# merbanan/rtl_433

Measured on NVIDIA H100. Metric: IQ MS/s end-to-end demod+slice, higher is better.
Workload: dtype u8/int16/int32 fixed point

## Files before the change

rtl_433_b200/csrc/r433b_api.cu:

```cuda
#include <algorithm>
#include <cmath>
#include <cstdio>
#include <cstdlib>
#include <chrono>
#include <cstring>
#include <exception>
#include <atomic>
#include <mutex>
#include <string>
#include <thread>
#include <vector>

#include "../../include/r433b.h"
#include "../../include/r433b_abi.h"
#include "r433b_kernels.cuh"
#include "r433b_host.hpp"
#include "r433b_pulses.hpp"
#include "r433b_analyze.cuh"
#include "r433b_analyze_host.hpp"
#include "r433b_grab.cuh"

using namespace r433b;

#ifdef R433B_SIMT_EMU
// ... 859 lines not shown
    ctx->timing.front_redone = counters[4];
    ctx->timing.front_repairs = counters[5];
    ctx->timing.idle_skipped = counters[6];
    ctx->timing.idle_rewalks = counters[7];
    ctx->timing.chain_folds = counters[8];
    ctx->timing.chain_fm_rebuilds = counters[9];
    cudaEventElapsedTime(&ctx->timing.total_ms, ctx->ev[0], ctx->ev[3]);
    ctx->timing.d2h_ms = 0;
    ctx->timing.detect_launches = detect_launches;
    ctx->processed = true;
    finish_chain();
    return R433B_OK;
}

}

int r433b_process(r433b_ctx *ctx, r433b_batch const *b) { return process_iq(ctx, b, nullptr, nullptr); }

int r433b_chain_create(r433b_ctx *ctx, uint32_t n_streams, r433b_chain **out)
{
    if (!ctx || !out || !n_streams) return fail(ctx, R433B_EINVAL, "r433b_chain_create: null argument or no streams");
    *out = nullptr;
    CU(cudaSetDevice(ctx->device));
    r433b_chain *ch = new (std::nothrow) r433b_chain();
    if (!ch) return R433B_ENOMEM;
    ch->ctx = ctx;
    ctx->chains.push_back(ch);
    ch->n = n_streams;
    ch->open.assign(n_streams, 0);
    ch->next.assign(n_streams, 0);
    size_t const n = n_streams;
    for (auto [buf, bytes] : {std::pair<DevBuf *, size_t>{&ch->d_state, n * sizeof(StreamState)}, {&ch->d_state_copy, n * sizeof(StreamState)},
                              {&ch->d_train, n * kTrainInts * sizeof(int)}, {&ch->d_train_copy, n * kTrainInts * sizeof(int)},
                              {&ch->d_flags, 2 * n}, {&ch->d_base, n * sizeof(uint64_t)}})
        if (int r = dev_reserve(ctx, *buf, bytes)) {
            r433b_chain_destroy(ch);
            return r;
        }
    *out = ch;
    return R433B_OK;
}

void r433b_chain_destroy(r433b_chain *ch)
{
    if (!ch) return;
    if (r433b_ctx *ctx = ch->ctx) {
        ctx->chains.erase(std::remove(ctx->chains.begin(), ctx->chains.end(), ch), ctx->chains.end());
        cudaSetDevice(ctx->device);
        chain_free_device(ch);
    }
    delete ch;
}

int r433b_process_chained(r433b_ctx *ctx, r433b_batch const *b, r433b_chain *chain, uint8_t const *last)
{
    if (!chain || !chain->ctx) return fail(ctx, R433B_EINVAL, "r433b_process_chained: no chain, or its context is gone");
    return process_iq(ctx, b, chain, last);
}

int r433b_chain_base(r433b_chain const *chain, uint32_t stream, uint64_t *first_sample)
{
    if (!chain || !first_sample || stream >= chain->n) return R433B_EINVAL;
    *first_sample = stream < chain->base.size() ? chain->base[stream] : 0;
    return R433B_OK;
}

int r433b_get_counts(r433b_ctx const *ctx, uint64_t out[4])
{
    if (!ctx || !out) return R433B_EINVAL;
    if (!ctx->processed) return R433B_ESTATE;
    out[0] = ctx->n_pkgs;
    out[1] = ctx->n_events;
    out[2] = ctx->event_bytes;
    out[3] = ctx->n_samples;
    return R433B_OK;
}

int r433b_get_timing(r433b_ctx const *ctx, r433b_timing *out)
{
    if (!ctx || !out) return R433B_EINVAL;
    *out = ctx->timing;
    return R433B_OK;
}

int r433b_fetch(r433b_ctx *ctx, r433b_results *out)
{
    if (!ctx || !out) return R433B_EINVAL;
    if (!ctx->processed) return fail(ctx, R433B_ESTATE, "r433b_fetch before r433b_process");
    CU(cudaSetDevice(ctx->device));
    cudaStream_t const st = 0;
    uint32_t const n_devs = (uint32_t)ctx->devs.size();
    size_t pk_bytes = (size_t)ctx->n_pkgs * sizeof(r433b_package);
    size_t pool_bytes = (size_t)ctx->pool_used * sizeof(int);
    size_t pair_bytes = (size_t)ctx->n_pkgs * n_devs * sizeof(r433b_pair);
    CU(cudaEventRecord(ctx->ev[4], st));
    if (int r = host_reserve(ctx, ctx->h_pkgs, pk_bytes + 16)) return r;
    if (int r = host_reserve(ctx, ctx->h_ppool, pool_bytes + 16)) return r;
    if (int r = host_reserve(ctx, ctx->h_gpool, pool_bytes + 16)) return r;
    if (int r = host_reserve(ctx, ctx->h_pairs, pair_bytes + 16)) return r;
    if (int r = host_reserve(ctx, ctx->h_events, ctx->event_bytes + 16)) return r;
    if (!ctx->d2h_done) {
        if (pk_bytes) CU(cudaMemcpyAsync(ctx->h_pkgs.p, ctx->d_pkgs.p, pk_bytes, cudaMemcpyDeviceToHost, st));
        if (pool_bytes) {
            CU(cudaMemcpyAsync(ctx->h_ppool.p, ctx->d_ppool.p, pool_bytes, cudaMemcpyDeviceToHost, st));
            CU(cudaMemcpyAsync(ctx->h_gpool.p, ctx->d_gpool.p, pool_bytes, cudaMemcpyDeviceToHost, st));
        }
        if (pair_bytes && ctx->d_pairs.p) CU(cudaMemcpyAsync(ctx->h_pairs.p, ctx->d_pairs.p, pair_bytes, cudaMemcpyDeviceToHost, st));
        if (ctx->event_bytes) CU(cudaMemcpyAsync(ctx->h_events.p, ctx->d_arena.p, ctx->event_bytes, cudaMemcpyDeviceToHost, st));
        ctx->d2h_done = true;
    }
    CU(cudaEventRecord(ctx->ev[5], st));
    CU(cudaEventSynchronize(ctx->ev[5]));
    cudaEventElapsedTime(&ctx->timing.d2h_ms, ctx->ev[4], ctx->ev[5]);
    r433b_package *pk = (r433b_package *)ctx->h_pkgs.p;
    if (!ctx->fetched) {
        std::vector<uint32_t> &ix = ctx->dev_index;
        ix.resize(ctx->n_pkgs);
        for (uint32_t i = 0; i < ctx->n_pkgs; ++i) ix[i] = i;
        std::sort(ix.begin(), ix.end(), [pk](uint32_t a, uint32_t b) {
            return pk[a].stream != pk[b].stream ? pk[a].stream < pk[b].stream : pk[a].seq < pk[b].seq;
        });
        std::vector<r433b_package> sorted(ctx->n_pkgs);
        for (uint32_t i = 0; i < ctx->n_pkgs; ++i) sorted[i] = pk[ix[i]];
        if (ctx->n_pkgs) memcpy(pk, sorted.data(), (size_t)ctx->n_pkgs * sizeof(r433b_package));
        ctx->analyzed = false;
        ctx->p_events.assign(ctx->n_pkgs, 0);
        ctx->dispatched.assign(ctx->batch.n_streams, 0);
    }
    ctx->fetched = true;
    out->n_packages = ctx->n_pkgs;
    out->n_devices = n_devs;
    out->packages = pk;
    out->pulse_pool = (int32_t const *)ctx->h_ppool.p;
    out->gap_pool = (int32_t const *)ctx->h_gpool.p;
    out->pairs = (r433b_pair const *)ctx->h_pairs.p;
    out->events = (uint8_t const *)ctx->h_events.p;
    out->event_bytes = ctx->event_bytes;
    out->n_events = ctx->n_events;
    out->n_samples = ctx->n_samples;
    out->n_gated = ctx->n_gated;
    return R433B_OK;
}

int r433b_copy_stage(r433b_ctx *ctx, uint32_t stream, int16_t *am, int16_t *fm, uint64_t max_samples)
{
    if (!ctx || !am || !fm) return R433B_EINVAL;
    if (!ctx->processed || !ctx->batch.want_stages) return fail(ctx, R433B_ESTATE, "no stage arrays kept (batch.want_stages)");
    if (stream >= ctx->batch.n_streams) return fail(ctx, R433B_EINVAL, "stream out of range");
    CU(cudaSetDevice(ctx->device));
    uint64_t SS = ctx->batch.sample_format;
    uint64_t first = ctx->offsets[stream] / SS;
    uint64_t n = ctx->lengths[stream] / SS;
    if (n > max_samples) n = max_samples;
    if (n) {
        CU(cudaMemcpy(am, (int16_t const *)ctx->d_am.p + ctx->am_offsets[stream], n * sizeof(int16_t), cudaMemcpyDeviceToHost));
        CU(cudaMemcpy(fm, (int16_t const *)ctx->d_fm.p + first, n * sizeof(int16_t), cudaMemcpyDeviceToHost));
    }
    return (int)std::min<uint64_t>(n, 0x7fffffff);
}


int r433b_event_to_bitbuffer(uint8_t const *ev, uint32_t pair_bytes, uint32_t index, struct bitbuffer *out,
        uint32_t *consumed)
{
    return event_to_bitbuffer(ev, pair_bytes, index, out, consumed);
}

float r433b_package_file_pos(r433b_ctx const *ctx, r433b_results const *res, uint32_t package)
{
    if (!ctx || !res || package >= res->n_packages) return 0.0f;
    if (ctx->pulse_mode) return 0.0f;
    r433b_package const &k = res->packages[package];
    uint64_t SS = ctx->batch.sample_format;
    uint64_t bytes = ctx->lengths[k.stream] + (ctx->chained ? ctx->chain_base[k.stream] * SS : 0);
    uint32_t bb = ctx->batch.block_bytes;
    uint64_t n_blocks = (bytes + bb - 1) / bb;
    if (n_blocks == 0) return 0.0f;
    uint64_t blk = (uint64_t)k.block < n_blocks ? (uint64_t)k.block : n_blocks - 1;
    unsigned long n_read = (unsigned long)std::min<uint64_t>(bb, bytes - blk * bb);
    float pos = ((float)(int)blk * bb + n_read) / ctx->batch.samp_rate / (int)SS;
    return pos;
}

int r433b_package_to_pulse_data(r433b_ctx const *ctx, r433b_results const *res, uint32_t package, struct pulse_data *pd)
{
    if (!ctx || !res || !pd || package >= res->n_packages) return R433B_EINVAL;
    r433b_package const &k = res->packages[package];
    memset(pd, 0, sizeof(*pd));
    if (ctx->pulse_mode) {
        if (k.end_pos >= ctx->pulse_meta.size()) return R433B_EINVAL;
        PulseSet::Meta const &m = ctx->pulse_meta[k.end_pos];
        pd->sample_rate = m.rate;
        pd->num_pulses = m.num_pulses;
        memcpy(pd->pulse, res->pulse_pool + k.pulse_off, k.pulse_count * sizeof(int));
        memcpy(pd->gap, res->gap_pool + k.pulse_off, k.pulse_count * sizeof(int));
        pd->fsk_f1_est = m.fsk_f1_est;
        pd->fsk_f2_est = m.fsk_f2_est;
        pd->freq1_hz = m.freq1_hz;
        pd->freq2_hz = m.freq2_hz;
        return R433B_OK;
    }
    pd->offset = k.offset;
    pd->sample_rate = ctx->batch.samp_rate;
    pd->start_ago = k.start_ago;
    pd->end_ago = k.end_ago;
    pd->num_pulses = k.num_pulses;
    memcpy(pd->pulse, res->pulse_pool + k.pulse_off, k.pulse_count * sizeof(int));
    memcpy(pd->gap, res->gap_pool + k.pulse_off, k.pulse_count * sizeof(int));
    pd->ook_low_estimate = k.ook_low_estimate;
    pd->ook_high_estimate = k.ook_high_estimate;
    pd->fsk_f1_est = k.fsk_f1_est;
    pd->fsk_f2_est = k.fsk_f2_est;
    float hi = pd->ook_high_estimate > 0 ? pd->ook_high_estimate : 1;
    float lo = pd->ook_low_estimate > 0 ? pd->ook_low_estimate : 1;
    int const max_high = ctx->lv.max_high;
    float top = hi < max_high ? hi : max_high;
    float asnr = top / lo;
    uint32_t rate = ctx->batch.samp_rate, center = ctx->batch.center_frequency;
    float off1 = (float)pd->fsk_f1_est / INT16_MAX * rate / 2.0f;
    float off2 = (float)pd->fsk_f2_est / INT16_MAX * rate / 2.0f;
    pd->freq1_hz = off1 + center;
    pd->freq2_hz = off2 + center;
    pd->centerfreq_hz = center;
    pd->depth_bits = ctx->batch.sample_format * 4;
    if (ctx->batch.sample_format == 2 && !ctx->use_mag) {
        pd->range_db = 42.1442f;
        pd->rssi_db = 10.0f * log10f(hi) - 42.1442f;
        pd->noise_db = 10.0f * log10f(lo) - 42.1442f;
        pd->snr_db = 10.0f * log10f(asnr);
    } else {
        pd->range_db = 84.2884f;
        pd->rssi_db = 20.0f * log10f(hi) - 84.2884f;
        pd->noise_db = 20.0f * log10f(lo) - 84.2884f;
        pd->snr_db = 20.0f * log10f(asnr);
    }
    return R433B_OK;
}

}

namespace {

template <class PerEvent, class PerPair>
int replay_stream(r433b_ctx *ctx, r433b_results const *res, uint32_t stream, PerEvent &&per_event, PerPair &&per_pair)
{
    if (!ctx || !res) return R433B_EINVAL;
    if (!ctx->fetched) return fail(ctx, R433B_ESTATE, "dispatch before fetch");
    uint32_t const n_devs = res->n_devices;
    r433b_package const *begin = std::lower_bound(res->packages, res->packages + res->n_packages, stream,
            [](r433b_package const &k, uint32_t s) { return k.stream < s; });
    static thread_local struct pulse_data pd;
    static thread_local struct bitbuffer bits;
    for (r433b_package const *k = begin; k != res->packages + res->n_packages && k->stream == stream; ++k) {
        uint32_t pi = (uint32_t)(k - res->packages);
        r433b_package_to_pulse_data(ctx, res, pi, &pd);
        int p_events = 0;
        unsigned next = 0;
        for (unsigned prio = 0; !p_events && prio < 0xffffffffu; prio = next) {
            next = 0xffffffffu;
            for (uint32_t dv = 0; dv < n_devs; ++dv) {
                unsigned dp = ctx->devs[dv].priority;
                if (dp > prio && dp < next) next = dp;
                if (dp != prio) continue;
                if (!device_takes((int)ctx->devs[dv].modulation, k->type)) continue;
                r433b_pair const &pr = res->pairs[(size_t)k->first_pair + dv];
                per_pair(dv, pr);
                uint32_t at = 0;
                for (uint32_t e = 0; e < pr.events; ++e) {
                    uint32_t used = 0;
                    int rc = r433b_event_to_bitbuffer(res->events + pr.offset + at, pr.bytes - at, 0, &bits, &used);
                    if (rc) return fail(ctx, rc, "corrupt event stream");
                    at += used;
                    int ret = per_event(pi, dv, &pd, &bits);
                    if (ret < -4) return fail(ctx, R433B_EINVAL, "decoder returned an invalid code (< -4)");
                    if (ret > 0) p_events += ret;
                }
            }
        }
        if (pi < ctx->p_events.size()) ctx->p_events[pi] = (uint32_t)p_events;
    }
    if (stream < ctx->dispatched.size()) ctx->dispatched[stream] = 1;
    return R433B_OK;
}

}

extern "C" {

int r433b_stream_digest(r433b_ctx *ctx, r433b_results const *res, uint32_t stream, uint64_t *digest)
{
    if (!ctx || !res || !digest) return R433B_EINVAL;
    if (!ctx->fetched) return fail(ctx, R433B_ESTATE, "digest before fetch");
    uint64_t h = 1469598103934665603ull;
    auto mix = [&](uint32_t w) {
        h ^= w;
        h *= 1099511628211ull;
    };
    auto mix_words = [&](void const *ptr, size_t n_words) {
        uint32_t const *w = (uint32_t const *)ptr;
        for (size_t i = 0; i < n_words; ++i) mix(w[i]);
    };
    r433b_package const *begin = std::lower_bound(res->packages, res->packages + res->n_packages, stream,
            [](r433b_package const &k, uint32_t s) { return k.stream < s; });
    for (r433b_package const *k = begin; k != res->packages + res->n_packages && k->stream == stream; ++k) {
        uint32_t const hdr[] = {k->seq, (uint32_t)k->type, (uint32_t)k->block, (uint32_t)k->offset, (uint32_t)(k->offset >> 32),
                                ctx->pulse_mode ? 0u : (uint32_t)k->end_pos, ctx->pulse_mode ? 0u : (uint32_t)(k->end_pos >> 32), k->start_ago, k->end_ago, k->num_pulses,
                                k->pulse_count, (uint32_t)k->ook_low_estimate, (uint32_t)k->ook_high_estimate,
                                (uint32_t)k->fsk_f1_est, (uint32_t)k->fsk_f2_est};
        mix_words(hdr, sizeof(hdr) / 4);
        mix_words(res->pulse_pool + k->pulse_off, k->pulse_count);
        mix_words(res->gap_pool + k->pulse_off, k->pulse_count);
        for (uint32_t dv = 0; dv < res->n_devices; ++dv) {
            r433b_pair const &pr = res->pairs[(size_t)k->first_pair + dv];
            mix(pr.bytes);
            mix(pr.events);
            mix(pr.gated_single);
            mix(pr.gated_multi);
            if (pr.bytes) mix_words(res->events + pr.offset, pr.bytes / 4);
        }
    }
    *digest = h;
    return R433B_OK;
}

int r433b_dispatch(r433b_ctx *ctx, r433b_results const *res, uint32_t stream, r433b_event_fn fn, void *user)
{
    if (!fn) return R433B_EINVAL;
    return replay_stream(ctx, res, stream, [&](uint32_t pk, uint32_t dv, struct pulse_data *pd, struct bitbuffer *bits) {
        return fn(user, pk, dv, pd, bits);
    }, [](uint32_t, r433b_pair const &) {});
}

int r433b_dispatch_r_devices(r433b_ctx *ctx, r433b_results const *res, uint32_t stream, struct r_device *const *devs,
        uint32_t n)
{
    if (!devs || !res || n != res->n_devices) return R433B_EINVAL;
    return replay_stream(ctx, res, stream, [&](uint32_t, uint32_t dv, struct pulse_data *, struct bitbuffer *bits) {
        struct r_device *d = devs[dv];
        int ret = 0;
        if (d->decode_fn) ret = d->decode_fn(d, bits);
        d->decode_events += 1;
        if (ret > 0) {
            d->decode_ok += 1;
            d->decode_messages += ret;
        } else if (ret >= -4) {
            d->decode_fails[-ret] += 1;
            ret = 0;
        }
        return ret;
    }, [&](uint32_t dv, r433b_pair const &pr) {
        if (!(pr.gated_single | pr.gated_multi) || ctx->gates.size() != n) return;
        struct r_device *d = devs[dv];
        r433b_gate const &g = ctx->gates[dv];
        d->decode_events += pr.gated_single + pr.gated_multi;
        d->decode_fails[-g.code_single] += pr.gated_single;
        d->decode_fails[-g.code_multi] += pr.gated_multi;
    });
}

}

extern "C" {

int r433b_dispatch_r_devices_parallel(r433b_ctx *ctx, r433b_results const *res, struct r_device *const *const *dev_sets,
        uint32_t n_devs, uint32_t n_sets)
{
    if (!ctx || !res || !dev_sets || !n_sets || n_devs != res->n_devices) return R433B_EINVAL;
    if (!ctx->fetched) return fail(ctx, R433B_ESTATE, "dispatch before fetch");
    uint32_t const n_streams = res->n_packages ? res->packages[res->n_packages - 1].stream + 1 : 0;
    std::atomic<int> first_error{0};
    auto work = [&](uint32_t w) {
        for (uint32_t s = w; s < n_streams && !first_error.load(std::memory_order_relaxed); s += n_sets) {
            int rc = r433b_dispatch_r_devices(ctx, res, s, dev_sets[w], n_devs);
            if (rc) {
                int expected = 0;
                first_error.compare_exchange_strong(expected, rc);
            }
        }
    };
    std::vector<std::thread> pool;
    for (uint32_t w = 1; w < n_sets; ++w) pool.emplace_back(work, w);
    work(0);
    for (auto &t : pool) t.join();
    return first_error.load();
}

}


extern "C" {

r433b_pulses *r433b_pulses_create(void) { return new (std::nothrow) r433b_pulses(); }

void r433b_pulses_destroy(r433b_pulses *ps) { delete ps; }

void r433b_pulses_clear(r433b_pulses *ps)
{
    if (!ps) return;
    ps->set = PulseSet();
}

int r433b_pulses_load_ook(r433b_pulses *ps, uint32_t stream, char const *text, size_t len, uint32_t samp_rate)
{
    if (!ps || (!text && len) || !samp_rate) return R433B_EINVAL;
    return load_ook_text(ps->set, stream, text, len, samp_rate);
}

int r433b_pulses_load_rfraw(r433b_pulses *ps, uint32_t stream, char const *line)
{
    if (!ps || !line) return R433B_EINVAL;
    if (!rfraw_is(line)) return 0;
    static thread_local struct pulse_data d;
    memset(&d, 0, sizeof(d));
    rfraw_append(&d, line);
    ps->set.add(stream, &d);
    return 1;
}

int r433b_pulses_add(r433b_pulses *ps, uint32_t stream, struct pulse_data const *pd)
{
    if (!ps || !pd) return R433B_EINVAL;
    ps->set.add(stream, pd);
    return 1;
}

uint32_t r433b_pulses_count(r433b_pulses const *ps) { return ps ? (uint32_t)ps->set.pk.size() : 0; }

int r433b_pulses_get(r433b_pulses const *ps, uint32_t index, struct pulse_data *out)
{
    if (!ps || !out || index >= ps->set.pk.size()) return R433B_EINVAL;
    ps->set.get(index, out);
    return R433B_OK;
}

size_t r433b_format_ook(struct pulse_data const *pd, char const *received, char *buf, size_t cap)
{
    return pd ? format_ook(pd, received, buf, cap) : 0;
}

size_t r433b_format_ook_header(char const *created, char *buf, size_t cap) { return format_ook_header(created, buf, cap); }

size_t r433b_format_vcd(struct pulse_data const *pd, int ch_id, char *buf, size_t cap)
{
    return pd ? format_vcd(pd, ch_id, buf, cap) : 0;
}

size_t r433b_format_vcd_header(uint32_t sample_rate, char const *date, char *buf, size_t cap)
{
    return format_vcd_header(sample_rate, date, buf, cap);
}

void r433b_dump_logic_u8(uint8_t *buf, uint64_t len, uint64_t buf_offset, struct pulse_data const *pd, uint8_t bits)
{
    if (buf && pd) dump_logic_u8(buf, len, buf_offset, pd, bits);
}

int r433b_process_pulses(r433b_ctx *ctx, r433b_pulses const *ps)
{
    if (!ctx || !ps) return fail(ctx, R433B_EINVAL, "null argument");
    CU(cudaSetDevice(ctx->device));
    PulseSet const &set = ps->set;
    uint32_t const n = (uint32_t)set.pk.size();
    uint32_t const n_devs = (uint32_t)ctx->devs.size();
    if ((uint64_t)n * n_devs > 0xffffffffull)
        return fail(ctx, R433B_EOVERFLOW, "packages x devices exceeds the 32-bit pair index (r433b_package.first_pair)");
    ctx->processed = ctx->fetched = false;
    ctx->d2h_done = false;
    ctx->pulse_mode = true;
    ctx->grab_planned = false;
    ctx->pulse_meta = set.pk;
    ctx->batch = r433b_batch{};
    ctx->batch.sample_format = 2;
    ctx->offsets.clear();
    ctx->lengths.clear();
    cudaStream_t const st = 0;

    std::vector<uint32_t> order(n);
    for (uint32_t i = 0; i < n; ++i) order[i] = i;
    std::stable_sort(order.begin(), order.end(), [&](uint32_t a, uint32_t b) { return set.pk[a].rate < set.pk[b].rate; });
    std::vector<r433b_package> hp(n);
    std::vector<int32_t> pp, gp;
    pp.reserve(set.pulse.size());
    gp.reserve(set.gap.size());
    std::vector<uint32_t> rates;
    std::vector<GroupRange> ranges;
    for (uint32_t j = 0; j < n; ++j) {
        PulseSet::Meta const &m = set.pk[order[j]];
        r433b_package &k = hp[j];
        memset(&k, 0, sizeof(k));
        k.stream = m.stream;
        k.seq = m.seq;
        k.type = m.type;
        k.end_pos = order[j];
        k.num_pulses = m.num_pulses;
        k.pulse_off = (uint32_t)pp.size();
        k.pulse_count = m.count;
        k.fsk_f1_est = m.fsk_f1_est;
        k.fsk_f2_est = m.fsk_f2_est;
        k.first_pair = j * n_devs;
        pp.insert(pp.end(), set.pulse.begin() + m.first, set.pulse.begin() + m.first + m.count);
        gp.insert(gp.end(), set.gap.begin() + m.first, set.gap.begin() + m.first + m.count);
        if (rates.empty() || rates.back() != m.rate) {
            rates.push_back(m.rate);
            ranges.push_back(GroupRange{});
            ranges.back().pkg_begin = j;
        }
        ranges.back().pkg_end = j + 1;
    }
    for (uint32_t rate : rates)
        if (!rate) return fail(ctx, R433B_EINVAL, "a package has sample_rate 0");

    ctx->n_pkgs = n;
    ctx->pool_used = (unsigned)pp.size();
    ctx->n_samples = 0;
    ctx->event_bytes = ctx->n_events = ctx->n_gated = 0;
    ctx->timing = r433b_timing{};
    if (n) {
        if (int r = dev_reserve(ctx, ctx->d_pkgs, (size_t)n * sizeof(r433b_package))) return r;
        if (int r = dev_reserve(ctx, ctx->d_ppool, pp.size() * sizeof(int) + 16)) return r;
        if (int r = dev_reserve(ctx, ctx->d_gpool, gp.size() * sizeof(int) + 16)) return r;
        CU(cudaMemcpyAsync(ctx->d_pkgs.p, hp.data(), (size_t)n * sizeof(r433b_package), cudaMemcpyHostToDevice, st));
        CU(cudaMemcpyAsync(ctx->d_ppool.p, pp.data(), pp.size() * sizeof(int), cudaMemcpyHostToDevice, st));
        CU(cudaMemcpyAsync(ctx->d_gpool.p, gp.data(), gp.size() * sizeof(int), cudaMemcpyHostToDevice, st));
        CU(cudaStreamSynchronize(st));
    }
    if (n && n_devs) {
        size_t const arena_min = ctx->min_caps[2] ? ctx->min_caps[2] : (size_t)(1u << 20);
        if (ctx->arena_cap < arena_min) ctx->arena_cap = arena_min;
        if (int r = upload_slicer_tables(ctx, rates, st)) return r;
        if (int r = slice_ranges(ctx, ranges, n, st)) return r;
        ctx->timing.total_ms = ctx->timing.slice_ms;
    }
    ctx->processed = true;
    return R433B_OK;
}

}



namespace {

uint32_t package_rate(r433b_ctx const *ctx, r433b_package const &k)
{
    if (ctx->pulse_mode && k.end_pos < ctx->pulse_meta.size()) return ctx->pulse_meta[k.end_pos].rate;
    return ctx->batch.samp_rate;
}

}

extern "C" {

int r433b_analyze(r433b_ctx *ctx, r433b_results const *res)
{
    if (!ctx || !res) return R433B_EINVAL;
    if (!ctx->fetched) return fail(ctx, R433B_ESTATE, "r433b_analyze before r433b_fetch");
    CU(cudaSetDevice(ctx->device));
    uint32_t const n = ctx->n_pkgs;
    ctx->an.assign(n, r433b_analysis{});
    ctx->an_guess.assign(n, r433b_guess{});
    ctx->an_text.assign(n, std::string());
    ctx->an_pairs.assign(n, r433b_pair{});
    ctx->an_events.clear();
    ctx->analyzed = true;
    if (!n) return R433B_OK;
    cudaStream_t const st = 0;
    if (int r = dev_reserve(ctx, ctx->d_an, (size_t)n * sizeof(r433b_analysis))) return r;
    AnalyzeParams ap{};
    ap.pkgs = (r433b_package const *)ctx->d_pkgs.p;
    ap.n_pkgs = n;
    ap.pulse_pool = (int const *)ctx->d_ppool.p;
    ap.gap_pool = (int const *)ctx->d_gpool.p;
    ap.out = (r433b_analysis *)ctx->d_an.p;
    unsigned const grid = (unsigned)(((uint64_t)n * 5 + kAnalyzeThreads - 1) / kAnalyzeThreads);
    R4_LAUNCH(k_analyze, grid, kAnalyzeThreads, 0, st, ap);
    CU(cudaGetLastError());
    CU(cudaMemcpyAsync(ctx->an.data(), ctx->d_an.p, (size_t)n * sizeof(r433b_analysis), cudaMemcpyDeviceToHost, st));
    CU(cudaStreamSynchronize(st));
    std::vector<SlicerParams> sp(n);
    std::vector<int> last_gap(n, -1);
    static thread_local struct pulse_data pd;
    std::vector<char> buf(1 << 16);
    bool any = false;
    for (uint32_t i = 0; i < n; ++i) {
        uint32_t const di = ctx->dev_index[i];
        r433b_package_to_pulse_data(ctx, res, i, &pd);
        r433b_guess g{};
        size_t len = analysis_finish(&pd, res->packages[i].type, ctx->an[di], &g, buf.data(), buf.size());
        if (len >= buf.size()) {
            buf.resize(len + 1);
            len = analysis_finish(&pd, res->packages[i].type, ctx->an[di], &g, buf.data(), buf.size());
        }
        ctx->an_text[di].assign(buf.data(), len);
        ctx->an_guess[di] = g;
        sp[di] = SlicerParams{};
        if (g.modulation && g.sliced) {
            r433b_device d{};
            d.modulation = g.modulation;
            d.short_width = g.short_width;
            d.long_width = g.long_width;
            d.reset_limit = g.reset_limit;
            d.gap_limit = g.gap_limit;
            d.sync_width = g.sync_width;
            d.tolerance = g.tolerance;
            sp[di] = scale_device(d, package_rate(ctx, res->packages[i]));
            last_gap[di] = g.last_gap;
            any = true;
        }
    }
    if (!any) return R433B_OK;
    if (int r = dev_reserve(ctx, ctx->d_an_dev, (size_t)n * sizeof(SlicerParams))) return r;
    if (int r = dev_reserve(ctx, ctx->d_an_gap, (size_t)n * sizeof(int))) return r;
    if (int r = dev_reserve(ctx, ctx->d_an_pairs, (size_t)n * sizeof(r433b_pair))) return r;
    CU(cudaMemcpyAsync(ctx->d_an_dev.p, sp.data(), (size_t)n * sizeof(SlicerParams), cudaMemcpyHostToDevice, st));
    CU(cudaMemcpyAsync(ctx->d_an_gap.p, last_gap.data(), (size_t)n * sizeof(int), cudaMemcpyHostToDevice, st));
    CU(cudaMemsetAsync(ctx->d_an_pairs.p, 0, (size_t)n * sizeof(r433b_pair), st));
    OwnSliceParams op{};
    op.pkgs = ap.pkgs;
    op.n_pkgs = n;
    op.pulse_pool = ap.pulse_pool;
    op.gap_pool = (int *)ctx->d_gpool.p;
// ... 321 lines not shown
```

rtl_433_b200/csrc/r433b_host.hpp:

```cpp
#pragma once
#include <algorithm>
#include <cmath>
#include <cstdint>
#include <cstring>
#include <vector>

#include "../../include/r433b.h"
#include "../../include/r433b_abi.h"
#include "r433b_core.cuh"
#include "r433b_slice.cuh"

namespace r433b {

inline Levels compute_levels(int use_mag, float level_limit, float min_level, float min_snr)
{
    Levels lv;
    if (use_mag) {
        lv.fixed_high = level_limit < 0.0 ? (int)(powf(10, (level_limit + 84.2884f) / 20.0f)) : 0;
        lv.min_high = (int)(powf(10, (min_level + 84.2884f) / 20.0f));
        lv.ratio = (int)(0.5 + powf(10, min_snr / 20.0f));
    } else {
        lv.fixed_high = level_limit < 0.0 ? (int)(powf(10, (level_limit + 42.1442f) / 10.0f)) : 0;
        lv.min_high = (int)(powf(10, (min_level + 42.1442f) / 10.0f));
        lv.ratio = (int)(0.5 + powf(10, min_snr / 10.0f));
    }
    lv.max_high = (int)(powf(10, (0 + 42.1442f) / 10.0f));
    return lv;
}

inline void fm_coeffs(int cs16, uint32_t rate, float low_pass, int &a1, int &b0)
{
    if (low_pass > 1e4f)
        low_pass = low_pass / rate;
    else if (low_pass >= 1.0f)
        low_pass = 1e6f / low_pass / rate;
    double ita = 1.0 / tan(M_PI_2 * low_pass);
    if (!cs16) {
        double gain = 1.0 / (1.0 + ita) / 2;
        a1 = (int)((ita - 1.0) * gain * 32768);
        b0 = (int)(gain * 32768);
    } else {
        double gain = 1.0 / (1.0 + ita);
        a1 = (int)((ita - 1.0) * gain * (1 << 30));
        b0 = (int)(gain * (1 << 30));
    }
}

inline SlicerParams scale_device(r433b_device const &d, uint32_t rate)
{
    SlicerParams t{};
    float per_us = rate / 1.0e6f;
    t.modulation = (int)d.modulation;
    t.s_short = d.short_width * per_us;
    t.s_long = d.long_width * per_us;
    t.s_reset = d.reset_limit * per_us;
    t.s_gap = d.gap_limit * per_us;
    t.s_sync = d.sync_width * per_us;
    t.s_tol = d.tolerance * per_us;
    bool bad3 = (d.short_width > 0 && t.s_short <= 0) || (d.long_width > 0 && t.s_long <= 0)
            || (d.reset_limit > 0 && t.s_reset <= 0);
    bool bad6 = bad3 || (d.gap_limit > 0 && t.s_gap <= 0) || (d.sync_width > 0 && t.s_sync <= 0)
            || (d.tolerance > 0 && t.s_tol <= 0);
    t.ok = (bad6 ? 0 : 1) | (bad3 ? 0 : 2);
    if ((int)d.modulation == kModOokRzi) {
        t.s_gap = t.s_sync = t.s_tol = 0;
    }
    t.f_short = d.short_width > 0.0f ? 1.0f / (d.short_width * per_us) : 0;
    t.f_long = d.long_width > 0.0f ? 1.0f / (d.long_width * per_us) : 0;
    t.priority = d.priority;
    return t;
}


inline std::vector<unsigned> slice_list(std::vector<r433b_device> const &devs, int package_type)
{
    std::vector<unsigned> v;
    for (unsigned i = 0; i < (unsigned)devs.size(); ++i)
        if (device_takes((int)devs[i].modulation, package_type)) v.push_back(i);
    std::sort(v.begin(), v.end(), [&](unsigned a, unsigned c) {
        r433b_device const &x = devs[a], &y = devs[c];
        if (x.modulation != y.modulation) return x.modulation < y.modulation;
        if (x.reset_limit != y.reset_limit) return x.reset_limit < y.reset_limit;
        if (x.short_width != y.short_width) return x.short_width < y.short_width;
        return a < c;
    });
    return v;
}


inline int event_to_bitbuffer(uint8_t const *ev8, uint32_t pair_bytes, uint32_t index, struct bitbuffer *out,
        uint32_t *consumed)
{
    if (!ev8 || !out || (pair_bytes & 3)) return -1;
    uint32_t const *ev = reinterpret_cast<uint32_t const *>(ev8);
    uint32_t const total = pair_bytes / 4;
    uint32_t pos = 0;
    for (uint32_t i = 0;; ++i) {
        if (pos + 1 > total) return -1;
        uint32_t h = ev[pos];
        uint32_t num_rows = h & 0x7f, dirty = (h >> 7) & 1, free_row = (h >> 8) & 0xff, len = h >> 16;
        if (len < 1 || pos + len > total) return -1;
        if (i == index) {
            memset(out, 0, sizeof(*out));
            out->num_rows = (uint16_t)num_rows;
            out->free_row = (uint16_t)free_row;
            uint32_t q = pos + 1;
            uint32_t const end = pos + len;
            uint8_t *flat = &out->bb[0][0];
            for (uint32_t r = 0; r < num_rows && r < R433B_BITBUF_ROWS; ++r) {
                if (q + 1 > end) return -1;
                uint32_t bits = ev[q] & 0xffff, syncs = ev[q] >> 16;
                q += 1;
                uint32_t words = (bits + 31) / 32;
                if (dirty && r + 1 == num_rows) words = ev[end - 1];
                if (q + words > end) return -1;
                out->bits_per_row[r] = (uint16_t)bits;
                out->syncs_before_row[r] = (uint16_t)syncs;
                size_t at = (size_t)r * R433B_BITBUF_COLS;
                size_t room = sizeof(out->bb) - at;
                size_t nb = (size_t)words * 4;
                memcpy(flat + at, ev + q, nb < room ? nb : room);
                q += words;
            }
            if (consumed) *consumed = (pos + len) * 4;
            return 0;
        }
        pos += len;
    }
}

}
```

rtl_433_b200/csrc/r433b_slice.cuh:

```cuda
#pragma once
#include <stdint.h>
#include "r433b_core.cuh"

namespace r433b {

constexpr int kBbRows = 50;
constexpr int kBbCols = 128;

#ifdef __CUDA_ARCH__
R4_HD float fmul(float a, float b) { return __fmul_rn(a, b); }
R4_HD float fadd(float a, float b) { return __fadd_rn(a, b); }
R4_HD float fdiv(float a, float b) { return __fdiv_rn(a, b); }
R4_HD double dadd(double a, double b) { return __dadd_rn(a, b); }
R4_HD double dmul(double a, double b) { return __dmul_rn(a, b); }
#else
R4_HD float fmul(float a, float b) { volatile float r = a * b; return r; }
R4_HD float fadd(float a, float b) { volatile float r = a + b; return r; }
R4_HD float fdiv(float a, float b) { volatile float r = a / b; return r; }
R4_HD double dadd(double a, double b) { volatile double r = a + b; return r; }
R4_HD double dmul(double a, double b) { volatile double r = a * b; return r; }
#endif

struct SlicerParams {
    int modulation;
    int ok;
    int s_short, s_long, s_reset, s_gap, s_sync, s_tol;
    float f_short, f_long;
    unsigned priority;
    int gate;
};


R4_HD uint32_t bswap32(uint32_t v)
{
#ifdef __CUDA_ARCH__
    return __byte_perm(v, 0, 0x0123);
#else
    return (v >> 24) | ((v >> 8) & 0xff00u) | ((v << 8) & 0xff0000u) | (v << 24);
#endif
}

#ifndef R4_SLICE_WINDOW
#define R4_SLICE_WINDOW 16
#endif
constexpr unsigned kSliceWindow = R4_SLICE_WINDOW;
static_assert(kSliceWindow >= 8 && (kSliceWindow & (kSliceWindow - 1)) == 0, "the window is a power of two of >= 1 sector");
struct NoWindow { static constexpr bool kOn = false; };

template <class Win>
R4_HD unsigned window_slide(uint32_t *out, unsigned wb, unsigned at)
{
    unsigned const b = (at + 8 - kSliceWindow) & ~7u;
    unsigned const end = b < wb + kSliceWindow ? b : wb + kSliceWindow;
    for (unsigned s = wb; s < end; s += 8) {
        uint32_t v[8];
#pragma unroll
        for (int k = 0; k < 8; ++k) v[k] = Win::slot((s + k) % kSliceWindow);
#ifdef __CUDA_ARCH__
        reinterpret_cast<uint4 *>(out + s)[0] = make_uint4(v[0], v[1], v[2], v[3]);
        reinterpret_cast<uint4 *>(out + s)[1] = make_uint4(v[4], v[5], v[6], v[7]);
#else
        for (int k = 0; k < 8; ++k) out[s + k] = v[k];
#endif
    }
    return b;
}

template <class Win = NoWindow>
struct EventWriterT {
    uint32_t *out;
    unsigned limit;
    unsigned wb;

    unsigned pos;
    unsigned committed;
    unsigned events;
    unsigned ev_start;
    unsigned num_rows, free_row;
    unsigned row0_bits;
    unsigned row_hdr;
    unsigned bits, syncs;
    unsigned row_hw;
    uint32_t acc;
    bool dirty;
    unsigned gate;
    unsigned max_bits;
    unsigned gated1, gatedN;

    R4_HD void init(uint32_t *o, unsigned region_words = 0, unsigned gate_bits = 0)
    {
        out = o;
        limit = region_words;
        wb = 0;
        pos = committed = 0;
        events = 0;
        gate = gate_bits;
        gated1 = gatedN = 0;
        reset_event();
    }

    R4_HD void reset_event()
    {
        pos = committed;
        ev_start = committed;
        num_rows = free_row = 0;
        row0_bits = 0;
        row_hdr = 0;
        bits = syncs = row_hw = 0;
        acc = 0;
        dirty = false;
        max_bits = 0;
        if constexpr (Win::kOn) {
            if (committed < wb) {
                unsigned const b = committed & ~7u;
                for (unsigned q = b; q < committed; ++q) Win::slot(q % kSliceWindow) = out[q];
                wb = b;
            }
        }
    }

    R4_HD void put(unsigned at, uint32_t v)
    {
        if (!out || at >= limit) return;
        if constexpr (Win::kOn) {
            if (at >= wb + kSliceWindow) wb = window_slide<Win>(out, wb, at);
            if (at >= wb) {
                Win::slot(at % kSliceWindow) = v;
                return;
            }
        }
        out[at] = v;
    }

    R4_HD uint32_t get(unsigned at) const
    {
        if constexpr (Win::kOn) {
            if (at >= wb) return Win::slot(at % kSliceWindow);
        }
        return out[at];
    }

    R4_HD unsigned first_row_bits() const { return num_rows <= 1 ? bits : row0_bits; }
    R4_HD unsigned last_row_bits() const { return bits; }

    R4_HD void open_row()
    {
        row_hdr = pos;
        pos += 1;
        bits = syncs = row_hw = 0;
        acc = 0;
    }

    R4_HD void flush_word()
    {
        unsigned w = (bits - 1) >> 5;
        unsigned at = row_hdr + 1 + w;
        if (out && at < limit) {
            uint32_t v = bswap32(acc);
            if (w < row_hw) v |= get(at);
            put(at, v);
        }
        if (w + 1 > row_hw) row_hw = w + 1;
        acc = 0;
    }

    R4_HD void close_row()
    {
        if (bits & 31) flush_word();
        put(row_hdr, bits | (syncs << 16));
        pos = row_hdr + 1 + row_hw;
    }

    R4_HD void first_row()
    {
        if (num_rows == 0) {
            ev_start = pos;
            pos += 1;
            num_rows = free_row = 1;
            open_row();
        }
    }

    R4_HD void add_bits(int value, int count)
    {
        first_row();
        {
            unsigned const p = bits & 31, in_row = bits & (kBbCols * 8 - 1);
            if ((unsigned)count <= 32 - p && (in_row != 0 || bits == 0) && bits < 60000u) {
                if (value) acc |= (0xffffffffu >> (32 - count)) << (32 - p - count);
                bits += (unsigned)count;
                if ((bits & 31) == 0) flush_word();
                return;
            }
        }
        while (count > 0) {
            if (bits == 65535u) return;
            if (bits > 0 && (bits & (kBbCols * 8 - 1)) == 0) {
                if (free_row < (unsigned)kBbRows)
                    free_row++;
                else
                    return;
            }
            unsigned p = bits & 31;
            unsigned room = 32 - p;
            unsigned n = (unsigned)count < room ? (unsigned)count : room;
            if (bits + n > 65535u) n = 65535u - bits;
            if (value) acc |= (n == 32 ? 0xffffffffu : ((1u << n) - 1u)) << (room - n);
            bits += n;
            count -= (int)n;
            if ((bits & 31) == 0) flush_word();
        }
    }

    R4_HD void add_bit(int bit) { add_bits(bit, 1); }

    R4_HD void add_row()
    {
        first_row();
        if (free_row < (unsigned)kBbRows) {
            if (num_rows == 1) row0_bits = bits;
            if (bits > max_bits) max_bits = bits;
            close_row();
            free_row++;
            for (unsigned r = num_rows; r + 1 < free_row; ++r) {
                put(pos, 0);
                pos += 1;
            }
            num_rows = free_row;
            open_row();
        } else {
            if (bits & 31) flush_word();
            bits = 0;
            dirty = true;
            acc = 0;
        }
    }

    R4_HD void add_sync()
    {
        first_row();
        if (bits) add_row();
        syncs++;
    }

    R4_HD void emit()
    {
        if (num_rows == 0) {
            ev_start = pos;
            pos += 1;
        } else if ((bits > max_bits ? bits : max_bits) < gate) {
            if (num_rows == 1) gated1++; else gatedN++;
            reset_event();
            return;
        } else {
            close_row();
            if (dirty) {
                put(pos, row_hw);
                pos += 1;
            }
        }
        put(ev_start, num_rows | (dirty ? 0x80u : 0u) | (free_row << 8) | ((pos - ev_start) << 16));
        committed = pos;
        events++;
        reset_event();
    }
};
using EventWriter = EventWriterT<>;


struct PulseView {
    int const *pulse;
    int const *gap;
    unsigned n;
};

enum {
    kModOokMc = 3, kModOokPcm = 4, kModOokPpm = 5, kModOokPwm = 6, kModOokPiwmRaw = 8, kModOokDmc = 9,
    kModOokOsv1 = 10, kModOokPiwmDc = 11, kModOokNrzs = 12, kModOokRzi = 13,
    kModFskPcm = 16, kModFskPwm = 17, kModFskMc = 18
};

R4_HD bool device_takes(int modulation, int package_type)
{
    if (package_type == 1) return modulation >= 3 && modulation <= 13 && modulation != 7;
    return modulation >= 16 && modulation <= 18;
}

R4_HD int iabs(int v) { return v < 0 ? -v : v; }
R4_HD bool within(int v, int nominal, int tol) { return v >= nominal - tol && v <= nominal + tol; }
R4_HD int symbol_at(PulseView const &p, unsigned k) { return (k & 1) ? p.gap[k >> 1] : p.pulse[k >> 1]; }

enum { kRowNone = 0, kRowAdd, kRowSync, kRowClear, kRowIfOpen };
enum { kEmitNone = 0, kEmitAlways, kEmitIfRows, kEmitIfData, kEmitIfRow0, kEmitElseRowIfOpen };
struct Step {
    int ones;
    int zeros;
    int row;
    int bit;
    int emit;
    bool stop_if_emitted, clear_after;
    int post_zeros;
};

struct SlicerState {
    unsigned k, total;
    int b0, b1, b2, b3, b4, b5;
    float f_short, f_long;
    int i0, i1, i2;
    int since;
    double edge;
    bool pending;
    int cv, cg;
};

R4_HD void slicer_advance(PulseView const &p, SlicerState &st, unsigned k)
{
    st.k = k;
    if (k < st.total) {
        st.cv = p.pulse[k];
        st.cg = p.gap[k];
    }
}

constexpr int kModAny = -1;
template <int MOD>
R4_HD int slicer_family(SlicerParams const &t)
{
    if (MOD != kModAny) return MOD;
    int const m = t.modulation;
    return m == kModFskPwm ? (int)kModOokPwm : m == kModFskPcm ? (int)kModOokPcm : m == kModFskMc ? (int)kModOokMc : m;
}

template <int MOD>
R4_HD bool slicer_begin0(PulseView const &p, SlicerParams const &t, SlicerState &st)
{
    st.k = 0;
    st.cv = st.cg = 0;
    st.total = p.n;
    st.since = 0;
    st.pending = false;
    int const big = 0x7fffffff;
    switch (slicer_family<MOD>(t)) {
    case kModOokPwm: {
        if (!(t.ok & 1)) return false;
        st.b4 = st.b5 = 0;
        if (t.s_tol > 0) {
            st.b0 = t.s_short - t.s_tol; st.b1 = t.s_short + t.s_tol;
            st.b2 = t.s_long - t.s_tol;  st.b3 = t.s_long + t.s_tol;
            if (t.s_sync > 0) { st.b4 = t.s_sync - t.s_tol; st.b5 = t.s_sync + t.s_tol; }
        } else if (t.s_sync <= 0) {
            st.b0 = 0; st.b1 = (t.s_short + t.s_long) / 2 + 1;
            st.b2 = st.b1 - 1; st.b3 = big;
        } else if (t.s_sync < t.s_short) {
            st.b4 = 0; st.b5 = (t.s_sync + t.s_short) / 2 + 1;
            st.b0 = st.b5 - 1; st.b1 = (t.s_short + t.s_long) / 2 + 1;
            st.b2 = st.b1 - 1; st.b3 = big;
        } else if (t.s_sync < t.s_long) {
            st.b0 = 0; st.b1 = (t.s_short + t.s_sync) / 2 + 1;
            st.b4 = st.b1 - 1; st.b5 = (t.s_sync + t.s_long) / 2 + 1;
            st.b2 = st.b5 - 1; st.b3 = big;
        } else {
            st.b0 = 0; st.b1 = (t.s_short + t.s_long) / 2 + 1;
            st.b2 = st.b1 - 1; st.b3 = (t.s_long + t.s_sync) / 2 + 1;
            st.b4 = st.b3 - 1; st.b5 = big;
        }
        return true;
    }
    case kModOokPpm: {
        if (!(t.ok & 1)) return false;
        st.b4 = st.b5 = 0;
        if (t.s_tol > 0) {
            st.b0 = t.s_short - t.s_tol; st.b1 = t.s_short + t.s_tol;
            st.b2 = t.s_long - t.s_tol;  st.b3 = t.s_long + t.s_tol;
            if (t.s_sync > 0) { st.b4 = t.s_sync - t.s_tol; st.b5 = t.s_sync + t.s_tol; }
        } else {
            st.b0 = 0;
            st.b1 = (t.s_short + t.s_long) / 2 + 1;
            st.b2 = st.b1 - 1;
            st.b3 = t.s_gap ? t.s_gap : t.s_reset;
        }
        return true;
    }
    case kModOokPcm: {
        if (!(t.ok & 1) || t.s_long == 0) return false;
        float f_short = t.f_short, f_long = t.f_long;
        int const gap_limit = t.s_gap ? t.s_gap : t.s_reset;
        int tol = t.s_tol;
        if (tol <= 0) tol = t.s_long / 4;
        bool const rz = t.s_short != t.s_long;
        int need = rz ? 4 : 12;
        int preamble = 0;
        unsigned const N = p.n;
        if (rz) {
            for (unsigned n = 0; n < N; ++n) {
                int sw = 0, lw = 0, cnt = 0;
                while (n < N && within(p.pulse[n], t.s_short, tol) && within(p.pulse[n] + p.gap[n], t.s_long, tol)) {
                    sw += p.pulse[n];
                    lw += p.pulse[n] + p.gap[n];
                    cnt++;
                    n++;
                }
                if (cnt >= need) {
                    f_long = fdiv((float)cnt, (float)lw);
                    f_short = fdiv((float)cnt, (float)sw);
                    need = cnt;
                    preamble = cnt;
                }
            }
            if (preamble == 0) {
                int sw = 0, lw = 0, cnt = 0;
                for (unsigned n = 0; n < N; ++n) {
                    if (within(p.pulse[n], t.s_short, tol) && within(p.pulse[n] + p.gap[n], t.s_long, tol)) {
                        sw += p.pulse[n];
                        lw += p.pulse[n] + p.gap[n];
                        cnt++;
                    }
                }
                if (cnt > 8) {
                    f_long = fdiv((float)cnt, (float)lw);
                    f_short = fdiv((float)cnt, (float)sw);
                }
            }
        } else {
            for (unsigned n = 0; n < N; ++n) {
                int wsum = 0, cnt = 0;
                while (n < N && (int)dadd((double)fmul((float)p.pulse[n], f_short), 0.5) == 1
                        && (int)dadd((double)fmul((float)p.gap[n], f_long), 0.5) == 1) {
                    wsum += p.pulse[n] + p.gap[n];
                    cnt += 2;
                    n++;
                }
                if (cnt >= need) {
                    f_short = f_long = fdiv((float)cnt, (float)wsum);
                    need = cnt;
                    preamble = cnt;
                }
            }
            if (preamble == 0) {
                int wsum = 0, cnt = 0;
                for (unsigned n = 0; n < N; ++n) {
                    if (within(p.pulse[n], t.s_short, tol)) { wsum += p.pulse[n]; cnt += 1; }
                    if (within(p.pulse[n], 2 * t.s_short, tol)) { wsum += p.pulse[n]; cnt += 2; }
                    if (within(p.gap[n], t.s_long, tol)) { wsum += p.gap[n]; cnt += 1; }
                    if (within(p.gap[n], 2 * t.s_long, tol)) { wsum += p.gap[n]; cnt += 2; }
                }
                if (cnt > 20) f_short = f_long = fdiv((float)cnt, (float)wsum);
            }
        }
        st.f_short = f_short;
        st.f_long = f_long;
        st.i0 = gap_limit;
        st.i1 = gap_limit / t.s_long;
        st.i2 = tol;
        return true;
    }
    case kModOokMc:
        if (!(t.ok & 1)) return false;
        st.edge = dmul((double)t.s_short, 1.5);
        st.i0 = t.s_short - t.s_tol;
        st.i1 = t.s_short * 2 + t.s_tol;
        st.pending = true;
        return true;
    case kModOokDmc: case kModOokPiwmRaw: case kModOokPiwmDc:
        if (!(t.ok & 1)) return false;
        st.total = p.n * 2;
        return true;
    case kModOokNrzs:
        return (t.ok & 1) && t.s_short != 0;
    case kModOokOsv1: {
        if (!(t.ok & 1)) return false;
        int const half_lo = t.s_short / 2, half_hi = t.s_short * 3 / 2, sync_lo = 2 * half_hi;
        int pre = 0;
        unsigned n;
        for (n = 0; n < p.n; ++n) {
            if (p.pulse[n] > half_lo && p.gap[n] > half_lo) {
                pre++;
                if (p.gap[n] > half_hi) break;
            } else {
                return false;
            }
        }
        if (pre != 12) return false;
        ++n;
        if (n >= (unsigned)kMaxPulses) return false;
        if (p.pulse[n] < sync_lo || p.gap[n] < sync_lo) return false;
        st.since = 0;
        if (p.gap[n] > p.pulse[n]) {
            st.since = 1;
            st.pending = true;
        }
        st.k = n + 1;
        st.i0 = half_hi;
        return true;
    }
    case kModOokRzi:
        if (!(t.ok & 2) || t.s_long == 0) return false;
        st.i0 = t.s_long - t.s_short;
        st.since = 1;
        return true;
    default:
        return false;
    }
}

template <int MOD>
R4_HD bool slicer_begin(PulseView const &p, SlicerParams const &t, SlicerState &st)
{
    if (!slicer_begin0<MOD>(p, t, st)) return false;
    slicer_advance(p, st, st.k);
    return true;
}

template <int MOD>
R4_HD Step slicer_step(PulseView const &p, SlicerParams const &t, SlicerState &st)
{
    Step s;
    s.ones = s.zeros = s.post_zeros = 0;
    s.row = kRowNone;
    s.bit = 0;
    s.emit = kEmitNone;
    s.stop_if_emitted = s.clear_after = false;
    unsigned const n = st.k;
    switch (slicer_family<MOD>(t)) {
    case kModOokPwm: {
        int v = st.cv, g = st.cg;
        if (v > st.b0 && v < st.b1) s.ones = 1;
        else if (v > st.b2 && v < st.b3) s.zeros = 1;
        else if (v > st.b4 && v < st.b5) s.row = kRowSync;
        else if (v <= st.b0) { }
        else s.row = kRowAdd;
        if (n == st.total - 1 || g > t.s_reset) s.emit = kEmitIfRows;
        else if (t.s_gap > 0 && g > t.s_gap) s.emit = kEmitElseRowIfOpen;
        slicer_advance(p, st, n + 1);
        break;
    }
    case kModOokPpm: {
        int g = st.cg;
        if (g > st.b0 && g < st.b1) s.zeros = 1;
        else if (g > st.b2 && g < st.b3) s.ones = 1;
        else if (g > st.b4 && g < st.b5) s.row = kRowSync;
        else if (g < t.s_reset) s.row = kRowAdd;
        if (n == st.total - 1 || g >= t.s_reset) s.emit = kEmitIfData;
        slicer_advance(p, st, n + 1);
        break;
    }
    case kModOokPcm: {
        int v = st.cv, g = st.cg;
        int highs = (int)fadd(fmul((float)v, st.f_short), 0.5f);
        int lows = (int)fadd(fmul((float)(g + t.s_short - t.s_long), st.f_long), 0.5f);
        if (lows > st.i1) lows = st.i1;
        s.ones = highs > 0 ? highs : 0;
        s.zeros = lows > 0 ? lows : 0;
        if (t.s_short != t.s_long && iabs(v - t.s_short) > st.i2) s.row = kRowClear;
        else if (g > st.i0 && g <= t.s_reset) s.row = kRowAdd;
        if (n == st.total - 1 || g > t.s_reset) s.emit = kEmitIfData;
        slicer_advance(p, st, n + 1);
        break;
    }
    case kModOokMc: {
        if (st.pending) {
            st.pending = false;
            s.zeros = 1;
            break;
        }
// ... 186 lines not shown
```

Measured before the change: 124,300.

## Compress short event rows into packed single-word encodings

Adds compact event encodings: rows of up to 16 bits are packed into a single header word, and single-row events become one word total. This shrinks the event buffer the GPU writes and transfers. The host decoder and digest expand the compact form back to the long form, so consumers and the digest see the same content. The cost is extra branching in the kernel's emit path and host-side re-expansion work during digest.

```diff
diff --git a/rtl_433_b200/csrc/r433b_api.cu b/rtl_433_b200/csrc/r433b_api.cu
--- a/rtl_433_b200/csrc/r433b_api.cu
+++ b/rtl_433_b200/csrc/r433b_api.cu
@@ -1185,6 +1185,7 @@
     };
     r433b_package const *begin = std::lower_bound(res->packages, res->packages + res->n_packages, stream,
             [](r433b_package const &k, uint32_t s) { return k.stream < s; });
+    std::vector<uint32_t> longform;
     for (r433b_package const *k = begin; k != res->packages + res->n_packages && k->stream == stream; ++k) {
         uint32_t const hdr[] = {k->seq, (uint32_t)k->type, (uint32_t)k->block, (uint32_t)k->offset, (uint32_t)(k->offset >> 32),
                                 ctx->pulse_mode ? 0u : (uint32_t)k->end_pos, ctx->pulse_mode ? 0u : (uint32_t)(k->end_pos >> 32), k->start_ago, k->end_ago, k->num_pulses,
@@ -1195,11 +1196,19 @@
         mix_words(res->gap_pool + k->pulse_off, k->pulse_count);
         for (uint32_t dv = 0; dv < res->n_devices; ++dv) {
             r433b_pair const &pr = res->pairs[(size_t)k->first_pair + dv];
-            mix(pr.bytes);
+            longform.clear();
+            uint32_t const *ev = reinterpret_cast<uint32_t const *>(res->events + pr.offset);
+            for (uint32_t pos = 0, total = pr.bytes / 4; pos < total;) {
+                EventHead const e = event_head(ev[pos]);
+                if (e.len < 1 || pos + e.len > total || event_long_form(ev + pos, e, longform))
+                    return fail(ctx, R433B_EINVAL, "corrupt event stream");
+                pos += e.len;
+            }
+            mix((uint32_t)longform.size() * 4);
             mix(pr.events);
             mix(pr.gated_single);
             mix(pr.gated_multi);
-            if (pr.bytes) mix_words(res->events + pr.offset, pr.bytes / 4);
+            mix_words(longform.data(), longform.size());
         }
     }
     *digest = h;
diff --git a/rtl_433_b200/csrc/r433b_host.hpp b/rtl_433_b200/csrc/r433b_host.hpp
--- a/rtl_433_b200/csrc/r433b_host.hpp
+++ b/rtl_433_b200/csrc/r433b_host.hpp
@@ -88,6 +88,48 @@
 }
 
 
+struct EventHead {
+    uint32_t num_rows, dirty, free_row, len;
+};
+
+inline EventHead event_head(uint32_t h)
+{
+    if ((h & 0xff) == 0xff) return {1, 0, 1, 1};
+    return {h & 0x7f, (h >> 7) & 1, (h >> 8) & 0xff, h >> 16};
+}
+
+template <class Row>
+inline int event_rows(uint32_t const *ev, EventHead const &e, Row &&row)
+{
+    uint32_t const end = e.len;
+    uint32_t const h = ev[0];
+    if ((h & 0xff) == 0xff) {
+        uint32_t const data = h >> 16, bits = (h >> 8) & 31;
+        if (bits > 16) return -1;
+        row(0u, bits, (h >> 13) & 7, &data, bits ? 1u : 0u);
+        return 1;
+    }
+    uint32_t q = 1;
+    for (uint32_t r = 0; r < e.num_rows && r < R433B_BITBUF_ROWS; ++r) {
+        if (q + 1 > end) return -1;
+        uint32_t const w = ev[q];
+        q += 1;
+        if (w >> 31) {
+            uint32_t const data = w & 0xffff, bits = (w >> 16) & 31;
+            if (bits > 16) return -1;
+            row(r, bits, (w >> 21) & 0x3ff, &data, bits ? 1u : 0u);
+            continue;
+        }
+        uint32_t const bits = w & 0xffff;
+        uint32_t words = (bits + 31) / 32;
+        if (e.dirty && r + 1 == e.num_rows) words = ev[end - 1];
+        if (q + words > end) return -1;
+        row(r, bits, w >> 16, ev + q, words);
+        q += words;
+    }
+    return (int)q;
+}
+
 inline int event_to_bitbuffer(uint8_t const *ev8, uint32_t pair_bytes, uint32_t index, struct bitbuffer *out,
         uint32_t *consumed)
 {
@@ -95,38 +137,43 @@
     uint32_t const *ev = reinterpret_cast<uint32_t const *>(ev8);
     uint32_t const total = pair_bytes / 4;
     uint32_t pos = 0;
+    EventHead e;
     for (uint32_t i = 0;; ++i) {
         if (pos + 1 > total) return -1;
-        uint32_t h = ev[pos];
-        uint32_t num_rows = h & 0x7f, dirty = (h >> 7) & 1, free_row = (h >> 8) & 0xff, len = h >> 16;
-        if (len < 1 || pos + len > total) return -1;
-        if (i == index) {
-            memset(out, 0, sizeof(*out));
-            out->num_rows = (uint16_t)num_rows;
-            out->free_row = (uint16_t)free_row;
-            uint32_t q = pos + 1;
-            uint32_t const end = pos + len;
-            uint8_t *flat = &out->bb[0][0];
-            for (uint32_t r = 0; r < num_rows && r < R433B_BITBUF_ROWS; ++r) {
-                if (q + 1 > end) return -1;
-                uint32_t bits = ev[q] & 0xffff, syncs = ev[q] >> 16;
-                q += 1;
-                uint32_t words = (bits + 31) / 32;
-                if (dirty && r + 1 == num_rows) words = ev[end - 1];
-                if (q + words > end) return -1;
-                out->bits_per_row[r] = (uint16_t)bits;
-                out->syncs_before_row[r] = (uint16_t)syncs;
-                size_t at = (size_t)r * R433B_BITBUF_COLS;
-                size_t room = sizeof(out->bb) - at;
-                size_t nb = (size_t)words * 4;
-                memcpy(flat + at, ev + q, nb < room ? nb : room);
-                q += words;
-            }
-            if (consumed) *consumed = (pos + len) * 4;
-            return 0;
-        }
-        pos += len;
+        e = event_head(ev[pos]);
+        if (e.len < 1 || pos + e.len > total) return -1;
+        if (i == index) break;
+        pos += e.len;
     }
+    memset(out, 0, sizeof(*out));
+    out->num_rows = (uint16_t)e.num_rows;
+    out->free_row = (uint16_t)e.free_row;
+    uint8_t *flat = &out->bb[0][0];
+    int const rc = event_rows(ev + pos, e, [&](uint32_t r, uint32_t bits, uint32_t syncs, uint32_t const *data, uint32_t words) {
+        out->bits_per_row[r] = (uint16_t)bits;
+        out->syncs_before_row[r] = (uint16_t)syncs;
+        size_t at = (size_t)r * R433B_BITBUF_COLS;
+        size_t room = sizeof(out->bb) - at;
+        size_t nb = (size_t)words * 4;
+        memcpy(flat + at, data, nb < room ? nb : room);
+    });
+    if (rc < 0) return -1;
+    if (consumed) *consumed = (pos + e.len) * 4;
+    return 0;
+}
+
+inline int event_long_form(uint32_t const *ev, EventHead const &e, std::vector<uint32_t> &out)
+{
+    size_t const at = out.size();
+    out.push_back(0);
+    int const q = event_rows(ev, e, [&](uint32_t, uint32_t bits, uint32_t syncs, uint32_t const *data, uint32_t words) {
+        out.push_back(bits | (syncs << 16));
+        out.insert(out.end(), data, data + words);
+    });
+    if (q < 0) return -1;
+    out.insert(out.end(), ev + q, ev + e.len);
+    out[at] = e.num_rows | (e.dirty << 7) | (e.free_row << 8) | ((uint32_t)(out.size() - at) << 16);
+    return 0;
 }
 
 }
diff --git a/rtl_433_b200/csrc/r433b_slice.cuh b/rtl_433_b200/csrc/r433b_slice.cuh
--- a/rtl_433_b200/csrc/r433b_slice.cuh
+++ b/rtl_433_b200/csrc/r433b_slice.cuh
@@ -166,6 +166,11 @@
 
     R4_HD void close_row()
     {
+        if (bits <= 16 && syncs < 1024 && !dirty) {
+            put(row_hdr, (bswap32(acc) & 0xffffu) | (bits << 16) | (syncs << 21) | 0x80000000u);
+            pos = row_hdr + 1;
+            return;
+        }
         if (bits & 31) flush_word();
         put(row_hdr, bits | (syncs << 16));
         pos = row_hdr + 1 + row_hw;
@@ -245,6 +250,7 @@
 
     R4_HD void emit()
     {
+        bool const one_word = num_rows == 1 && bits <= 16 && syncs < 8 && !dirty;
         if (num_rows == 0) {
             ev_start = pos;
             pos += 1;
@@ -252,6 +258,8 @@
             if (num_rows == 1) gated1++; else gatedN++;
             reset_event();
             return;
+        } else if (one_word) {
+            pos = ev_start + 1;
         } else {
             close_row();
             if (dirty) {
@@ -259,7 +267,8 @@
                 pos += 1;
             }
         }
-        put(ev_start, num_rows | (dirty ? 0x80u : 0u) | (free_row << 8) | ((pos - ev_start) << 16));
+        put(ev_start, one_word ? 0xffu | (bits << 8) | (syncs << 13) | (bswap32(acc) << 16)
+                               : num_rows | (dirty ? 0x80u : 0u) | (free_row << 8) | ((pos - ev_start) << 16));
         committed = pos;
         events++;
         reset_event();
```

New measurement: 132,600, median of 6. 6.7% higher.
